# Sahar-E/NeRF-and-DietNeRF

Hardware: AMD Instinct MI355X
Metric: rays/sec (coarse+fine) at 256x256, 64 coarse + 128 fine samples (higher is better)
Workload: dtype f16 (3-pass hi/lo split operands, f32 accumulate; fp32-class results)

## Files before the change

### nerf_and_dietnerf_amd/csrc/aux_kernels.hip

```cpp
#include "field_device.h"
#include "nerf_kernels.h"
#include "ray_box_device.h"
#include "sampling_device.h"

#include <algorithm>

namespace nerf {

struct RaygenArgs {
    float c[16];
    float tan_half;
    int H, W;
    long long ray_begin, ray_count;
    float* orig;
    float* dirs;
};

__global__ void raygen_kernel(const RaygenArgs a) {
    const long long t = (long long)blockIdx.x * blockDim.x + threadIdx.x;
    if (t >= a.ray_count) return;
    const long long ray = a.ray_begin + t;
    const int i = (int)(ray / a.W), j = (int)(ray % a.W);
    const float x_ndc = __fdiv_rn((float)j + 0.5f, (float)a.W);
    const float y_ndc = __fdiv_rn((float)i + 0.5f, (float)a.H);
    const float xs = __fsub_rn(__fmul_rn(2.0f, x_ndc), 1.0f);
    const float ys = __fsub_rn(1.0f, __fmul_rn(2.0f, y_ndc));
    const float xc = __fmul_rn(xs, a.tan_half);
    const float yc = __fmul_rn(ys, a.tan_half);
    float d[4];
#pragma unroll
    for (int r = 0; r < 4; ++r) {
        float s = __fadd_rn(__fmul_rn(a.c[r * 4 + 0], xc), __fmul_rn(a.c[r * 4 + 1], yc));
        s = __fadd_rn(s, __fmul_rn(a.c[r * 4 + 2], -1.0f));
        s = __fadd_rn(s, __fmul_rn(a.c[r * 4 + 3], 0.0f));
        d[r] = s;
    }
    reinterpret_cast<float4*>(a.dirs)[t] = make_float4(d[0], d[1], d[2], d[3]);
    if (a.orig) reinterpret_cast<float4*>(a.orig)[t] = make_float4(a.c[3], a.c[7], a.c[11], a.c[15]);
}

static float raygen_tan_half(float fov) { return (float)tan((double)(fov * 0.5f)); }

void launch_raygen(const float c2w_host[16], float fov, int H, int W, long long ray_begin,
                   long long ray_count, float* orig, float* dirs, hipStream_t stream) {
    if (ray_count <= 0) return;
    RaygenArgs a;
    for (int i = 0; i < 16; ++i) a.c[i] = c2w_host[i];
    a.tan_half = raygen_tan_half(fov);
    a.H = H; a.W = W; a.ray_begin = ray_begin; a.ray_count = ray_count; a.orig = orig; a.dirs = dirs;
    hipLaunchKernelGGL(raygen_kernel, dim3(blocks_for(ray_count)), dim3(kBs), 0, stream, a);
}

__global__ void rays_to_ndc_kernel(const float* orig, const float* dirs, long long N, float n, float two_n, float k,
                                   float* out_orig, float* out_dirs) {
    const long long t = (long long)blockIdx.x * blockDim.x + threadIdx.x;
    if (t >= N) return;
    const float4 o = reinterpret_cast<const float4*>(orig)[t];
    const float4 d = reinterpret_cast<const float4*>(dirs)[t];
    const float tn = -__fdiv_rn(__fadd_rn(n, o.z), d.z);
    const float px = __fadd_rn(o.x, __fmul_rn(tn, d.x));
    const float py = __fadd_rn(o.y, __fmul_rn(tn, d.y));
    const float pz = __fadd_rn(o.z, __fmul_rn(tn, d.z));
    const float rx = __fdiv_rn(px, pz), ry = __fdiv_rn(py, pz), e = __fdiv_rn(two_n, pz);
    const float sx = __fdiv_rn(d.x, d.z), sy = __fdiv_rn(d.y, d.z);
    reinterpret_cast<float4*>(out_orig)[t] = make_float4(-__fmul_rn(k, rx), -__fmul_rn(k, ry), __fadd_rn(1.0f, e), o.w);
    reinterpret_cast<float4*>(out_dirs)[t] =
        make_float4(-__fmul_rn(k, __fsub_rn(sx, rx)), -__fmul_rn(k, __fsub_rn(sy, ry)), -e, d.w);
}

void launch_rays_to_ndc(const float* orig, const float* dirs, long long N, float fov, float near_plane, float* out_orig,
                        float* out_dirs, hipStream_t stream) {
    if (N <= 0) return;
    const float k = (float)(1.0 / (double)raygen_tan_half(fov));
    hipLaunchKernelGGL(rays_to_ndc_kernel, dim3(blocks_for(N)), dim3(kBs), 0, stream, orig, dirs, N,
                       near_plane, 2.0f * near_plane, k, out_orig, out_dirs);
}

__global__ void ray_box_bounds_kernel(const BoxArgs bx, const float* __restrict__ orig, const float* __restrict__ dirs,
                                      long long N, float* __restrict__ bounds, int* __restrict__ narrowed) {
    const long long r = (long long)blockIdx.x * blockDim.x + threadIdx.x;
    if (r >= N) return;
    float a, b;
    const bool nar = ray_box_interval(bx, reinterpret_cast<const float4*>(orig)[r], reinterpret_cast<const float4*>(dirs)[r], &a, &b);
    reinterpret_cast<float2*>(bounds)[r] = nar ? make_float2(a, b) : make_float2(bx.near_b, bx.far_b);
    if (narrowed) narrowed[r] = nar ? 1 : 0;
}

void launch_ray_box_bounds(const SceneBox& box, float near_b, float far_b, const float* orig, const float* dirs, long long N,
                           float* bounds, int* narrowed, hipStream_t stream) {
    if (N <= 0) return;
    hipLaunchKernelGGL(ray_box_bounds_kernel, dim3(blocks_for(N)), dim3(kBs), 0, stream,
                       box_args(box, near_b, far_b), orig, dirs, N, bounds, narrowed);
}

struct GridArgs {
    BoxArgs bx;
    const uint32_t* bits;
    int R;
};

__device__ __forceinline__ float grid_plane(float lo, float cell, int k, float o, float d) {
    return __fdiv_rn(__fsub_rn(__fadd_rn(lo, __fmul_rn(cell, (float)k)), o), d);
}

__device__ __forceinline__ int ray_grid_interval(const GridArgs& g, const float4 o, const float4 d, float* a, float* b) {
    const BoxArgs& bx = g.bx;
    const int R = g.R;
    float a0, b0;
    const bool hit = ray_box_hit(bx, o, d, &a0, &b0);
    const bool box_narrowed = hit && (a0 > bx.near_b || b0 < bx.far_b);
    const float oo[3] = {o.x, o.y, o.z}, dd[3] = {d.x, d.y, d.z};
    *a = bx.near_b; *b = bx.far_b;
    if (!hit) return 0;
    float cell[3], tp[3];
    int idx[3], step[3], plane[3];
#pragma unroll
    for (int ax = 0; ax < 3; ++ax) {
        cell[ax] = __fdiv_rn(__fsub_rn(bx.hi[ax], bx.lo[ax]), (float)R);
        const float p = __fadd_rn(oo[ax], __fmul_rn(a0, dd[ax]));
        idx[ax] = grid_cell_index(p, bx.lo[ax], cell[ax], R);
        step[ax] = dd[ax] > 0.0f ? 1 : -1;
        plane[ax] = idx[ax] + (dd[ax] > 0.0f ? 1 : 0);
        tp[ax] = dd[ax] == 0.0f ? __builtin_huge_valf() : grid_plane(bx.lo[ax], cell[ax], plane[ax], oo[ax], dd[ax]);
    }
    float t = a0, ga = 0.f, gb = 0.f;
    bool found = false;
    const int max_steps = 3 * R + 3;
    for (int it = 0; it < max_steps; ++it) {
        int ax = 0;
        float tm = tp[0];
        if (tp[1] < tm) { ax = 1; tm = tp[1]; }
        if (tp[2] < tm) { ax = 2; tm = tp[2]; }
        float te = tm;
        if (te > b0) te = b0;
        if (te < t) te = t;
        const int bit = idx[0] + R * (idx[1] + R * idx[2]);
        if ((g.bits[bit >> 5] >> (bit & 31)) & 1u) {
            if (!found) { ga = t; found = true; }
            gb = te;
        }
        if (!(tm < b0)) break;
#pragma unroll
        for (int k = 0; k < 3; ++k)
            if (k == ax) {
                idx[k] += step[k];
                plane[k] += step[k];
                tp[k] = grid_plane(bx.lo[k], cell[k], plane[k], oo[k], dd[k]);
            }
        if (idx[0] < 0 || idx[0] >= R || idx[1] < 0 || idx[1] >= R || idx[2] < 0 || idx[2] >= R) break;
        t = te;
    }
    if (found && gb > ga && (ga > a0 || gb < b0)) { *a = ga; *b = gb; return 2; }
    if (box_narrowed) { *a = a0; *b = b0; return 1; }
    return 0;
}

__global__ void ray_grid_bounds_kernel(const GridArgs g, const float* __restrict__ orig, const float* __restrict__ dirs,
                                       long long N, float* __restrict__ bounds, int* __restrict__ state) {
    const long long r = (long long)blockIdx.x * blockDim.x + threadIdx.x;
    if (r >= N) return;
    float a, b;
    const int st = ray_grid_interval(g, reinterpret_cast<const float4*>(orig)[r], reinterpret_cast<const float4*>(dirs)[r], &a, &b);
    reinterpret_cast<float2*>(bounds)[r] = make_float2(a, b);
    if (state) state[r] = st;
}

void launch_ray_grid_bounds(const SceneBox& box, float near_b, float far_b, const uint32_t* bits, int R, const float* orig,
                            const float* dirs, long long N, float* bounds, int* state, hipStream_t stream) {
    if (N <= 0) return;
    GridArgs g;
    g.bx = box_args(box, near_b, far_b);
    g.bits = bits; g.R = R;
    hipLaunchKernelGGL(ray_grid_bounds_kernel, dim3(blocks_for(N)), dim3(kBs), 0, stream, g, orig, dirs, N,
                       bounds, state);
}

enum DepthSrc { kDepthHost, kDepthBox, kDepthBounds };
struct DepthRays {
    BoxArgs bx; const float* orig; const float* dirs;
    const float* bounds; const int* state;
};

template <bool LINDISP, int SRC>
__global__ void z_values_kernel(const DepthRays rays, DepthConsts k, long long N, int S, const float* __restrict__ u,
                                uint64_t seed, long long ray_base, float* __restrict__ z) {
    const long long m = (long long)blockIdx.x * blockDim.x + threadIdx.x;
    if (m >= N * S) return;
    const long long r = m / S;
    const int s = (int)(m - r * S);
    if constexpr (SRC == kDepthBox) {
        float a, b;
        if (ray_box_interval(rays.bx, reinterpret_cast<const float4*>(rays.orig)[r],
                             reinterpret_cast<const float4*>(rays.dirs)[r], &a, &b))
            k = depth_consts_of_interval<LINDISP>(a, b, S);
    } else if constexpr (SRC == kDepthBounds) {
        if (rays.state[r] != 0) {
            const float2 ab = reinterpret_cast<const float2*>(rays.bounds)[r];
            k = depth_consts_of_interval<LINDISP>(ab.x, ab.y, S);
        }
    }
    const float uu = u ? u[m] : philox_uniform(seed, (uint64_t)(ray_base + r), s, 0u);
    z[m] = stratified_depth<LINDISP>(k, s, S, uu);
}

static DepthConsts depth_consts_host(float near_b, float far_b, bool lindisp, int S) {
    if (lindisp)
        return {near_b, nextafterf(far_b, near_b), (float)(1.0 / (double)near_b),
                (float)(1.0 / (double)far_b - 1.0 / (double)near_b)};
    return {near_b, far_b, S > 1 ? (far_b - near_b) / (float)(S - 1) : 0.f, (float)((double)far_b - (double)near_b)};
}

void launch_z_values(float near_b, float far_b, bool lindisp, long long N, int S, const float* u, uint64_t seed,
                     long long ray_base, float* z, hipStream_t stream, const float* orig, const float* dirs,
                     const SceneBox* box, const float* bounds, const int* state) {
    if (N <= 0) return;
    using Kernel = void (*)(const DepthRays, DepthConsts, long long, int, const float*, uint64_t, long long, float*);
    static const Kernel kernels[3][2] = {{z_values_kernel<false, kDepthHost>, z_values_kernel<true, kDepthHost>},
                                         {z_values_kernel<false, kDepthBox>, z_values_kernel<true, kDepthBox>},
                                         {z_values_kernel<false, kDepthBounds>, z_values_kernel<true, kDepthBounds>}};
    const DepthSrc src = bounds && state ? kDepthBounds : box && orig && dirs ? kDepthBox : kDepthHost;
    DepthRays rays = {};
    if (src == kDepthBox) { rays.bx = box_args(*box, near_b, far_b); rays.orig = orig; rays.dirs = dirs; }
    if (src == kDepthBounds) { rays.bounds = bounds; rays.state = state; }
    hipLaunchKernelGGL(kernels[src][lindisp ? 1 : 0], dim3(blocks_for(N * S)), dim3(kBs), 0, stream, rays,
                       depth_consts_host(near_b, far_b, lindisp, S), N, S, u, seed, ray_base, z);
}

constexpr int kPdfWaves = 4;

__global__ __launch_bounds__(64 * kPdfWaves) void sample_pdf_kernel(
    const float* __restrict__ weights, const float* __restrict__ zin, long long N, int S, int Sf,
    const float* __restrict__ u, uint64_t seed, long long ray_base, float* __restrict__ z_new,
    float* __restrict__ z_merged) {
    extern __shared__ __attribute__((aligned(16))) float lds[];
    const int lane = threadIdx.x & 63;
    const int wave = threadIdx.x >> 6;
    const long long ray = (long long)blockIdx.x * kPdfWaves + wave;
    if (ray >= N) return;
    const int S4 = (S + 3) & ~3, Sf4 = (Sf + 3) & ~3, T = S + Sf, T4 = (T + 3) & ~3;
    const int per_wave = S4 + S4 + Sf4 + T4;
    float* cdf = lds + wave * per_wave;
    float* zc = cdf + S4;
    float* zn = zc + S4;
    float* za = zn + Sf4;
    const float* wr = weights + ray * S;
    const float* zr = zin + ray * S;
    ray_cdf(wr, zr, S, lane, cdf, zc, nullptr);
    const float kInf = __builtin_huge_valf();
    for (int k = lane; k < Sf4; k += 64) {
        if (k >= Sf) { zn[k] = kInf; continue; }
        const float uu = u ? u[ray * Sf + k] : philox_uniform(seed, (uint64_t)(ray_base + ray), k, 1u);
        zn[k] = inverse_cdf_draw(cdf, zc, S, uu).z;
    }
    __builtin_amdgcn_fence(__ATOMIC_ACQ_REL, "wavefront");
    __builtin_amdgcn_wave_barrier();
    for (int k = lane; k < Sf; k += 64) {
        const float v = zn[k];
        const int rank = stable_rank(zn, Sf4, v, k);
        if (z_new) z_new[ray * Sf + rank] = v;
        za[rank] = v;
    }
    if (z_merged) {
        __builtin_amdgcn_fence(__ATOMIC_ACQ_REL, "wavefront");
        __builtin_amdgcn_wave_barrier();
        bool bad = false;
        for (int s = lane; s + 1 < S; s += 64) bad |= zc[s + 1] < zc[s];
        if (!__any(bad)) {
            for (int k = lane; k < Sf; k += 64) {
                const float v = za[k];
                z_merged[ray * T + k + count_below(zc, S, v)] = v;
            }
            for (int j = lane; j < S; j += 64) {
                const float v = zc[j];
                z_merged[ray * T + j + count_not_above(za, Sf, v)] = v;
            }
        } else {
            for (int k = lane; k < T4; k += 64) if (k >= Sf) za[k] = k < T ? zc[k - Sf] : kInf;
            __builtin_amdgcn_fence(__ATOMIC_ACQ_REL, "wavefront");
            __builtin_amdgcn_wave_barrier();
            for (int k = lane; k < T; k += 64) {
                const float v = za[k];
                z_merged[ray * T + stable_rank(za, T4, v, k)] = v;
            }
        }
    }
}

size_t sample_pdf_lds_bytes(int S, int Sf) {
    const int S4 = (S + 3) & ~3, Sf4 = (Sf + 3) & ~3, T4 = (S + Sf + 3) & ~3;
    return (size_t)kPdfWaves * (S4 + S4 + Sf4 + T4) * sizeof(float);
}

void launch_sample_pdf(const float* weights, const float* z, long long N, int S, int Sf, const float* u,
                       uint64_t seed, long long ray_base, float* z_new, float* z_merged, hipStream_t stream) {
    if (N <= 0) return;
    const size_t lds = sample_pdf_lds_bytes(S, Sf);
    hipLaunchKernelGGL(sample_pdf_kernel, dim3((unsigned)((N + kPdfWaves - 1) / kPdfWaves)), dim3(64 * kPdfWaves),
                       lds, stream, weights, z, N, S, Sf, u, seed, ray_base, z_new, z_merged);
}

template <bool SIGMA_ONLY>
__global__ __launch_bounds__(256) void composite_kernel(const float* __restrict__ raw, const float* __restrict__ z,
                                                        long long N, int S, float* __restrict__ rgb,
                                                        float* __restrict__ weights, float* __restrict__ cumprod,
                                                        float* __restrict__ alpha_out, float* __restrict__ rgb_samples,
                                                        float* __restrict__ depth) {
    const int lane = threadIdx.x & 63;
    const long long r = (long long)blockIdx.x * 4 + (threadIdx.x >> 6);
    if (r >= N) return;
    const float4* rw = reinterpret_cast<const float4*>(raw) + r * S;
    const float* zr = z + r * S;
    float carry = 1.0f, c0 = 0.f, c1 = 0.f, c2 = 0.f, dep = 0.f;
    for (int s0 = 0; s0 < S; s0 += 64) {
        const int s = s0 + lane;
        const bool in = s < S;
        const float4 o = SIGMA_ONLY ? make_float4(0.f, 0.f, 0.f, in ? raw[r * S + s] : 0.f)
                                    : in ? rw[s] : make_float4(0.f, 0.f, 0.f, 0.f);
        const float zc = in ? zr[s] : 0.f;
        const CompositeTerms ct = composite_terms(o, zr, s, S);
        const float a = ct.alpha, r0 = ct.r0, r1 = ct.r1, r2 = ct.r2;
        const float om = 1.0f - a;
        const float oms = __int_as_float(__builtin_amdgcn_update_dpp(__float_as_int(1.0f), __float_as_int(om), 0x138, 0xf, 0xf, false));
        float T = lane == 0 ? carry : 1.0f;
        const int rounds = S - s0 < 64 ? S - s0 - 1 : 63;
        for (int k = 0; k < rounds; ++k) {
            const float Ts = __int_as_float(__builtin_amdgcn_update_dpp(__float_as_int(T), __float_as_int(T), 0x138, 0xf, 0xf, false));
            T = Ts * (lane == 0 ? 1.0f : oms);
        }
        const float w = a * T;
        if constexpr (SIGMA_ONLY) {
            if (in) weights[r * S + s] = w;
            carry = __shfl(T * om, 63);
            continue;
        }
        c0 += w * r0; c1 += w * r1; c2 += w * r2; dep += w * zc;
        if (in) {
            const long long m = r * S + s;
            if (weights) weights[m] = w;
            if (cumprod) cumprod[m] = T;
            if (alpha_out) alpha_out[m] = a;
            if (rgb_samples) { rgb_samples[m * 3 + 0] = r0; rgb_samples[m * 3 + 1] = r1; rgb_samples[m * 3 + 2] = r2; }
        }
        carry = __shfl(T * om, 63);
    }
    if constexpr (SIGMA_ONLY) return;
#pragma unroll
    for (int o = 32; o > 0; o >>= 1) {
        c0 += __shfl_xor(c0, o); c1 += __shfl_xor(c1, o); c2 += __shfl_xor(c2, o); dep += __shfl_xor(dep, o);
    }
    if (lane == 0) {
        if (rgb) { rgb[r * 3 + 0] = c0; rgb[r * 3 + 1] = c1; rgb[r * 3 + 2] = c2; }
        if (depth) depth[r] = dep;
    }
}

void launch_composite(const float* raw, const float* z, long long N, int S, float* rgb, float* weights,
                      float* cumprod, float* alpha, float* rgb_samples, float* depth, hipStream_t stream) {
    if (N <= 0) return;
    hipLaunchKernelGGL(composite_kernel<false>, dim3((unsigned)((N + 3) / 4)), dim3(256), 0, stream, raw, z, N, S,
                       rgb, weights, cumprod, alpha, rgb_samples, depth);
}

void launch_composite_weights(const float* sigma, const float* z, long long N, int S, float* weights, hipStream_t stream) {
    if (N <= 0) return;
    hipLaunchKernelGGL(composite_kernel<true>, dim3((unsigned)((N + 3) / 4)), dim3(256), 0, stream, sigma, z, N, S,
                       nullptr, weights, nullptr, nullptr, nullptr, nullptr);
}

__global__ void posenc_kernel(const float* __restrict__ x, long long M, int n_enc, int passthrough,
                              float* __restrict__ out) {
    const long long m = (long long)blockIdx.x * blockDim.x + threadIdx.x;
    if (m >= M) return;
    const int per = (passthrough ? 1 : 0) + 2 * n_enc;
    const float kPi = 3.1415927410125732f;
    for (int c = 0; c < 3; ++c) {
        const float v = x[m * 3 + c];
        float* o = out + m * (3 * per) + c * per;
        if (passthrough) *o++ = v;
        for (int k = 0; k < n_enc; ++k) {
            const float th = __fmul_rn(v, kPi * (float)(1 << k));
            o[2 * k] = sin_shifted(th, 0);
            o[2 * k + 1] = sin_shifted(th, 1);
        }
    }
}

void launch_posenc(const float* x, long long M, int n_enc, int passthrough, float* out, hipStream_t stream) {
    if (M <= 0) return;
    hipLaunchKernelGGL(posenc_kernel, dim3(blocks_for(M)), dim3(kBs), 0, stream, x, M, n_enc,
                       passthrough, out);
}

__device__ __forceinline__ float repack_weight(const float* __restrict__ blob, const float* __restrict__ scale, int32_t src) {
    const float w = blob[src];
    return scale ? __fmul_rn(w, scale[src]) : w;
}

template <class E>
__global__ void repack_kernel(const float* __restrict__ blob, const float* __restrict__ scale, const int32_t* __restrict__ idx,
                              E* __restrict__ out, size_t n, const int32_t* __restrict__ const_idx, float* __restrict__ cst) {
    const size_t i = (size_t)blockIdx.x * blockDim.x + threadIdx.x;
    if (i < n) {
        const int32_t t = idx[i];
        E v = (E)0.f;
        if constexpr (sizeof(E) == sizeof(float)) {
            if (t != 0) v = repack_weight(blob, scale, t - 1);
        } else if (t != 0) {
            const float w = repack_weight(blob, scale, (t >> 1) - 1);
            const E hi = (E)w;
            v = (t & 1) ? (E)(w - (float)hi) : hi;
        }
        out[i] = v;
    }
    if (const_idx && i < (size_t)kConstFloats) {
        const int32_t t = const_idx[i];
        cst[i] = t ? repack_weight(blob, scale, t - 1) : 0.f;
    }
}

void launch_repack(StreamElem elem, const float* blob, const float* scale, const int32_t* idx, void* out, size_t n,
                   const int32_t* const_idx, float* cst, hipStream_t s) {
    const dim3 grid((unsigned)((std::max(n, (size_t)kConstFloats) + 255) / 256)), block(256);
    if (elem == kElemF32) hipLaunchKernelGGL(repack_kernel<float>, grid, block, 0, s, blob, scale, idx, (float*)out, n, const_idx, cst);
    else if (elem == kElemBf16) hipLaunchKernelGGL(repack_kernel<__bf16>, grid, block, 0, s, blob, scale, idx, (__bf16*)out, n, const_idx, cst);
    else hipLaunchKernelGGL(repack_kernel<_Float16>, grid, block, 0, s, blob, scale, idx, (_Float16*)out, n, const_idx, cst);
}

}
```

### nerf_and_dietnerf_amd/csrc/sampling_device.h

```cpp
#pragma once
#include "nerf_device.h"

namespace nerf {

struct DepthConsts { float c0, c1, c2, c3; };

template <bool LINDISP>
__device__ __forceinline__ DepthConsts depth_consts_of_interval(float a, float b, int S) {
    DepthConsts k;
    k.c0 = a;
    if constexpr (LINDISP) {
        k.c1 = __int_as_float(__float_as_int(b) - 1);
        k.c2 = __fdiv_rn(1.0f, a);
        k.c3 = __fsub_rn(__fdiv_rn(1.0f, b), k.c2);
    } else {
        k.c1 = b;
        k.c3 = __fsub_rn(b, a);
        k.c2 = S > 1 ? __fdiv_rn(k.c3, (float)(S - 1)) : 0.f;
    }
    return k;
}

template <bool LINDISP>
__device__ __forceinline__ float stratified_depth(const DepthConsts& k, int s, int S, float u) {
    if constexpr (LINDISP) {
        const float top = (float)(s + 1);
        float v = __fadd_rn((float)s, u);
        if (v >= top) v = __int_as_float(__float_as_int(top) - 1);
        const float t = __fdiv_rn(v, (float)S);
        const float zz = __fdiv_rn(1.0f, __fadd_rn(k.c2, __fmul_rn(k.c3, t)));
        return fminf(fmaxf(zz, k.c0), k.c1);
    } else {
        float lin = __fadd_rn(k.c0, __fmul_rn(k.c2, (float)s));
        if (s == 0) lin = k.c0;
        if (s == S - 1 && S > 1) lin = k.c1;
        return __fadd_rn(lin, __fdiv_rn(__fmul_rn(u, k.c3), (float)S));
    }
}

__device__ __forceinline__ int count_below(const float* arr, int n, float v) {
    int lo = 0, hi = n;
    while (lo < hi) { const int mid = (lo + hi) >> 1; if (arr[mid] < v) lo = mid + 1; else hi = mid; }
    return lo;
}

__device__ __forceinline__ int count_not_above(const float* arr, int n, float v) {
    int lo = 0, hi = n;
    while (lo < hi) { const int mid = (lo + hi) >> 1; if (arr[mid] <= v) lo = mid + 1; else hi = mid; }
    return lo;
}

__device__ __forceinline__ int stable_rank(const float* arr, int n4, float v, int k) {
    int rank = 0;
    for (int i = 0; i < n4; i += 4) {
        const float4 o = *reinterpret_cast<const float4*>(arr + i);
        rank += (o.x < v || (o.x == v && i + 0 < k)) ? 1 : 0;
        rank += (o.y < v || (o.y == v && i + 1 < k)) ? 1 : 0;
        rank += (o.z < v || (o.z == v && i + 2 < k)) ? 1 : 0;
        rank += (o.w < v || (o.w == v && i + 3 < k)) ? 1 : 0;
    }
    return rank;
}

constexpr int kCdfChunks = 4;

__device__ __forceinline__ float ray_cdf(const float* __restrict__ wr, const float* __restrict__ zr, int S, int lane,
                                         float* cdf, float* zc, float* wv) {
    float den = 0.f;
    if (S <= 64 * kCdfChunks) {
        float wreg[kCdfChunks], creg[kCdfChunks];
#pragma unroll
        for (int c = 0; c < kCdfChunks; ++c) {
            const int s = lane + 64 * c;
            wreg[c] = s < S ? wr[s] : 0.f;
            if (s < S) { zc[s] = zr[s]; if (wv) wv[s] = wreg[c]; }
        }
        float sum = 0.f;
#pragma unroll
        for (int c = 0; c < kCdfChunks; ++c) {
            const int n = min(64, S - 64 * c);
            for (int i = 0; i < n; ++i) sum = __fadd_rn(sum, __shfl(wreg[c], i));
        }
        den = __fadd_rn(sum, 1e-7f);
        float acc = 0.f;
#pragma unroll
        for (int c = 0; c < kCdfChunks; ++c) {
            const float pdf = __fdiv_rn(wreg[c], den);
            const int n = min(64, S - 64 * c);
            creg[c] = 0.f;
            for (int i = 0; i < n; ++i) {
                acc = __fadd_rn(acc, __shfl(pdf, i));
                if (lane == i) creg[c] = acc;
            }
        }
#pragma unroll
        for (int c = 0; c < kCdfChunks; ++c) {
            const int s = lane + 64 * c;
            if (s < S) cdf[s] = creg[c];
        }
    } else {
        for (int s = lane; s < S; s += 64) {
            const float w = wr[s];
            cdf[s] = w; zc[s] = zr[s];
            if (wv) wv[s] = w;
        }
        __builtin_amdgcn_wave_barrier();
        __builtin_amdgcn_fence(__ATOMIC_ACQ_REL, "wavefront");
        if (lane == 0) {
            float sum = 0.f;
            for (int s = 0; s < S; ++s) sum = __fadd_rn(sum, cdf[s]);
            den = __fadd_rn(sum, 1e-7f);
            float acc = 0.f;
            for (int s = 0; s < S; ++s) {
                acc = __fadd_rn(acc, __fdiv_rn(cdf[s], den));
                cdf[s] = acc;
            }
        }
        den = __shfl(den, 0);
    }
    __builtin_amdgcn_fence(__ATOMIC_ACQ_REL, "wavefront");
    __builtin_amdgcn_wave_barrier();
    return den;
}

struct CdfDraw {
    float z, span, t, den;
    int b, t_bin;
    bool clamped;
};

__device__ __forceinline__ CdfDraw inverse_cdf_draw(const float* cdf, const float* zc, int S, float u) {
    CdfDraw d;
    const int idx = count_below(cdf, S, u);
    d.b = max(0, idx - 1);
    d.t_bin = min(S - 1, idx);
    const float c_lo = cdf[d.b], c_hi = cdf[d.t_bin];
    const int bz = min(max(d.b, 0), S - 2), tz = min(max(d.t_bin, 0), S - 2);
    const float z_lo = __fmul_rn(0.5f, __fadd_rn(zc[bz + 1], zc[bz]));
    const float z_hi = __fmul_rn(0.5f, __fadd_rn(zc[tz + 1], zc[tz]));
    d.den = __fsub_rn(c_hi, c_lo);
    d.clamped = d.den < 1e-5f;
    d.den = d.clamped ? 1e-5f : d.den;
    d.t = __fdiv_rn(__fsub_rn(u, c_lo), d.den);
    d.span = __fsub_rn(z_hi, z_lo);
    d.z = __fadd_rn(z_lo, __fmul_rn(d.t, d.span));
    return d;
}

struct CompositeTerms { float delta, sigma, e, alpha, r0, r1, r2; };

__device__ __forceinline__ float raw_sigmoid(float x) { return 1.0f / (1.0f + expf(-x)); }

__device__ __forceinline__ CompositeTerms composite_terms(const float4 o, const float* __restrict__ zr, int s, int S) {
    CompositeTerms c;
    c.delta = s + 1 < S ? zr[s + 1] - zr[s] : 1e9f;
    c.sigma = fmaxf(o.w, 0.f);
    c.e = s < S ? expf(-(c.sigma * c.delta)) : 1.0f;
    c.alpha = 1.0f - c.e;
    c.r0 = raw_sigmoid(o.x);
    c.r1 = raw_sigmoid(o.y);
    c.r2 = raw_sigmoid(o.z);
    return c;
}

}
```

Baseline: 1.817 million.

## Replace rank-counting sort in PDF sampling with wave-level bitonic sorts

The fine-sample sorting in the sample_pdf kernel used an O(n^2) stable-rank count over LDS per lane. It now uses a register-resident bitonic sort across the wavefront via shuffles when Sf fits in 128 keys, and an LDS bitonic sort otherwise, including the fallback merge path. This cuts the quadratic comparison work and LDS reads. The trade-off is that bitonic sort is not stable and needs many shuffle steps. Ties and NaN handling may also differ from the old stable ranking.

```diff
diff --git a/nerf_and_dietnerf_amd/csrc/aux_kernels.hip b/nerf_and_dietnerf_amd/csrc/aux_kernels.hip
--- a/nerf_and_dietnerf_amd/csrc/aux_kernels.hip
+++ b/nerf_and_dietnerf_amd/csrc/aux_kernels.hip
@@ -247,18 +247,30 @@
     const float* zr = zin + ray * S;
     ray_cdf(wr, zr, S, lane, cdf, zc, nullptr);
     const float kInf = __builtin_huge_valf();
-    for (int k = lane; k < Sf4; k += 64) {
-        if (k >= Sf) { zn[k] = kInf; continue; }
+    auto draw = [&](int k) {
         const float uu = u ? u[ray * Sf + k] : philox_uniform(seed, (uint64_t)(ray_base + ray), k, 1u);
-        zn[k] = inverse_cdf_draw(cdf, zc, S, uu).z;
-    }
-    __builtin_amdgcn_fence(__ATOMIC_ACQ_REL, "wavefront");
-    __builtin_amdgcn_wave_barrier();
-    for (int k = lane; k < Sf; k += 64) {
-        const float v = zn[k];
-        const int rank = stable_rank(zn, Sf4, v, k);
-        if (z_new) z_new[ray * Sf + rank] = v;
-        za[rank] = v;
+        return inverse_cdf_draw(cdf, zc, S, uu).z;
+    };
+    if (Sf <= kSortRegKeys) {
+        float v[2];
+#pragma unroll
+        for (int c = 0; c < 2; ++c) v[c] = lane + 64 * c < Sf ? draw(lane + 64 * c) : kInf;
+        wave_sort_regs(v[0], v[1], Sf, lane);
+#pragma unroll
+        for (int c = 0; c < 2; ++c) {
+            const int k = lane + 64 * c;
+            if (k < Sf) { za[k] = v[c]; if (z_new) z_new[ray * Sf + k] = v[c]; }
+        }
+    } else {
+        for (int k = lane; k < Sf; k += 64) zn[k] = draw(k);
+        __builtin_amdgcn_fence(__ATOMIC_ACQ_REL, "wavefront");
+        __builtin_amdgcn_wave_barrier();
+        wave_sort_lds(zn, Sf, lane);
+        for (int k = lane; k < Sf; k += 64) {
+            const float v = zn[k];
+            za[k] = v;
+            if (z_new) z_new[ray * Sf + k] = v;
+        }
     }
     if (z_merged) {
         __builtin_amdgcn_fence(__ATOMIC_ACQ_REL, "wavefront");
@@ -275,13 +287,11 @@
                 z_merged[ray * T + j + count_not_above(za, Sf, v)] = v;
             }
         } else {
-            for (int k = lane; k < T4; k += 64) if (k >= Sf) za[k] = k < T ? zc[k - Sf] : kInf;
+            for (int k = Sf + lane; k < T; k += 64) za[k] = zc[k - Sf];
             __builtin_amdgcn_fence(__ATOMIC_ACQ_REL, "wavefront");
             __builtin_amdgcn_wave_barrier();
-            for (int k = lane; k < T; k += 64) {
-                const float v = za[k];
-                z_merged[ray * T + stable_rank(za, T4, v, k)] = v;
-            }
+            wave_sort_lds(za, T, lane);
+            for (int k = lane; k < T; k += 64) z_merged[ray * T + k] = za[k];
         }
     }
 }
diff --git a/nerf_and_dietnerf_amd/csrc/sampling_device.h b/nerf_and_dietnerf_amd/csrc/sampling_device.h
--- a/nerf_and_dietnerf_amd/csrc/sampling_device.h
+++ b/nerf_and_dietnerf_amd/csrc/sampling_device.h
@@ -60,6 +60,48 @@
         rank += (o.w < v || (o.w == v && i + 3 < k)) ? 1 : 0;
     }
     return rank;
+}
+
+constexpr int kSortRegKeys = 128;
+
+__device__ __forceinline__ void wave_sort_regs(float& v0, float& v1, int n, int lane) {
+    for (int k = 2; k <= kSortRegKeys && (k >> 1) < n; k <<= 1) {
+        if (k == 128) {
+            const bool sw = v1 < v0;
+            const float lo = sw ? v1 : v0, hi = sw ? v0 : v1;
+            v0 = lo; v1 = hi;
+        }
+        for (int j = k == 128 ? 32 : k >> 1; j > 0; j >>= 1) {
+            const float o0 = __shfl_xor(v0, j), o1 = __shfl_xor(v1, j);
+            const bool lower = (lane & j) == 0;
+            const bool up0 = (lane & k) == 0;
+            const bool up1 = ((lane + 64) & k) == 0;
+            const bool sw0 = lower == up0 ? o0 < v0 : v0 < o0;
+            const bool sw1 = lower == up1 ? o1 < v1 : v1 < o1;
+            v0 = sw0 ? o0 : v0;
+            v1 = sw1 ? o1 : v1;
+        }
+    }
+}
+
+__device__ __forceinline__ void wave_sort_lds(float* arr, int n, int lane) {
+    int P = 1;
+    while (P < n) P <<= 1;
+    for (int k = 2; k <= P; k <<= 1) {
+        for (int j = k >> 1; j > 0; j >>= 1) {
+            const bool flip = j == (k >> 1);
+            for (int t = lane; t < (P >> 1); t += 64) {
+                const int off = t & (j - 1), base = (t - off) << 1;
+                const int lo = base + off, hi = flip ? base + k - 1 - off : lo + j;
+                if (hi < n) {
+                    const float a = arr[lo], b = arr[hi];
+                    if (b < a) { arr[lo] = b; arr[hi] = a; }
+                }
+            }
+            __builtin_amdgcn_fence(__ATOMIC_ACQ_REL, "wavefront");
+            __builtin_amdgcn_wave_barrier();
+        }
+    }
 }
 
 constexpr int kCdfChunks = 4;
```

After: 1.819 million (median of 6 runs). No clear change (+0.1%).
